# Luca96/carla-driving-rl-agent

Measured on AMD Instinct MI355X. Metric: PPO update-steps/sec (batch=256, 4x90x120x3 obs), higher is better.
Workload: dtype f32; 1 GPU; configs[1]: synthetic rollout buffer 256x4-frame 90x120x3 obs per GPU, full CARLANetwork fwd/bwd + PPO (re-sampled Beta, pathwise) / value loss + clip + Adam, fp32; per_gpu_batch=256, global_batch=256, parallelism=dp1, policy_loss=resampled (reference-faithful)

## Files before the change

carla-driving-rl-agent_amd/csrc/gemm_pw_bwd.hip:

```cpp
#include <stdlib.h>

#include "colreduce.h"

namespace cdrl {

typedef float f32x16 __attribute__((ext_vector_type(16)));
typedef __bf16 bf16x8 __attribute__((ext_vector_type(8)));
typedef __bf16 bf16x4 __attribute__((ext_vector_type(4)));
typedef uint32_t u32x2 __attribute__((ext_vector_type(2)));
typedef float f32x2 __attribute__((ext_vector_type(2)));

struct PwbArgs {
    View dz;
    int dz_shuffle;
    int act;
    const float* y;
    const float* stats;
    const float* coef;
    View a;
    const float* a_stats;
    const __bf16* Wp;
    int wp_ks;
    View da;
    float* qpart;
// ... 471 lines not shown
                int dc = shuffle_dst(a.dz.coff + c0 + h, a.dz_shuffle);
                if (dc + 1 >= a.dz.ld) {
                    dc -= 1;
                    hi_half[h] = true;
                }
                vo[h] = cok[h] ? (uint32_t)((4 * rg) * a.dz.ld + dc) * 2u : OOR;
            }
        } else {
            vo[0] = cok[0] ? (uint32_t)((4 * rg) * a.dz.ld + a.dz.coff + c0) * 2u : OOR;
            vo[1] = cok[2] ? (uint32_t)((4 * rg) * a.dz.ld + a.dz.coff + c0 + 2) * 2u : OOR;
        }
        voy[0] = cok[0] ? (uint32_t)((4 * rg) * N + c0) * 2u : OOR;
        voy[1] = cok[2] ? (uint32_t)((4 * rg) * N + c0 + 2) * 2u : OOR;
        const __amdgpu_buffer_rsrc_t rsD = __builtin_amdgcn_make_buffer_rsrc(a.dz.p, 0, (int)(Mtot * a.dz.ld * 2), 0x00020000);
        const __amdgpu_buffer_rsrc_t rsY = __builtin_amdgcn_make_buffer_rsrc(const_cast<float*>(a.y), 0, (int)(Mtot * N * 2), 0x00020000);
        const uint32_t rowD = (uint32_t)a.dz.ld * 2u, rowY = (uint32_t)N * 2u;
        const bool relu6 = a.act == ACT_RELU6;
        uint32_t rz[4][2], ry[4][2];
        auto load_row = [&](int t, int j) {
            const int64_t m0 = mbeg + (int64_t)t * BM;
            const uint32_t mu = (uint32_t)m0;
            const int left = (int)(mend - (m0 + 4 * rg));
            const uint32_t msk = j < left ? 0u : OOR;
#pragma unroll
            for (int h = 0; h < 2; ++h) {
                rz[j][h] = __builtin_amdgcn_raw_buffer_load_b32(rsD, (vo[h] + (uint32_t)j * rowD) | msk, mu * rowD, 0);
                ry[j][h] = __builtin_amdgcn_raw_buffer_load_b32(rsY, (voy[h] + (uint32_t)j * rowY) | msk, mu * rowY, 0);
            }
        };
        double cs[4] = {0.0, 0.0, 0.0, 0.0};
        auto store_tile = [&](int t) {
            const bool more = t + 1 < t1;
            const int left = (int)(mend - (mbeg + (int64_t)t * BM + 4 * rg));
            f32x2 cmean[2], cinv[2], csc[2], csh[2], ck1[2], ck2[2], ck3[2];
            {
                const float4 q0 = *reinterpret_cast<const float4*>(&cf[0 * NP + c0]), q1 = *reinterpret_cast<const float4*>(&cf[1 * NP + c0]);
                const float4 q2 = *reinterpret_cast<const float4*>(&cf[2 * NP + c0]), q3 = *reinterpret_cast<const float4*>(&cf[3 * NP + c0]);
                const float4 q4 = *reinterpret_cast<const float4*>(&cf[4 * NP + c0]), q5 = *reinterpret_cast<const float4*>(&cf[5 * NP + c0]);
                const float4 q6 = *reinterpret_cast<const float4*>(&cf[6 * NP + c0]);
                cmean[0] = f32x2{q0.x, q0.y}; cmean[1] = f32x2{q0.z, q0.w};
                cinv[0] = f32x2{q1.x, q1.y}; cinv[1] = f32x2{q1.z, q1.w};
                csc[0] = f32x2{q2.x, q2.y}; csc[1] = f32x2{q2.z, q2.w};
                csh[0] = f32x2{q3.x, q3.y}; csh[1] = f32x2{q3.z, q3.w};
                ck1[0] = f32x2{q4.x, q4.y}; ck1[1] = f32x2{q4.z, q4.w};
                ck2[0] = f32x2{q5.x, q5.y}; ck2[1] = f32x2{q5.z, q5.w};
                ck3[0] = f32x2{q6.x, q6.y}; ck3[1] = f32x2{q6.z, q6.w};
            }
            uint32_t hw[4][2];
            f32x2 ts[2] = {f32x2{0.0f, 0.0f}, f32x2{0.0f, 0.0f}};
#pragma unroll
            for (int j = 0; j < 4; ++j) {
                const bool rok = j < left;
                f32x2 dz2[2];
                if (SHUF) {
                    const f32x2 pa = widen(hi_half[0] ? rz[j][0] >> 16 : rz[j][0]), pb = widen(hi_half[1] ? rz[j][1] >> 16 : rz[j][1]);
                    dz2[0] = f32x2{pa[0], pb[0]};
                    dz2[1] = f32x2{pa[1], pb[1]};
                    if (!cok[2]) dz2[1][0] = 0.0f;
                    if (!cok[3]) dz2[1][1] = 0.0f;
                } else {
                    dz2[0] = widen(rz[j][0]);
                    dz2[1] = widen(rz[j][1]);
                }
                f32x2 vrow[2];
#pragma unroll
                for (int h = 0; h < 2; ++h) {
                    f32x2 d = dz2[h];
                    const f32x2 yv = widen(ry[j][h]);
                    if (relu6) {
                        const f32x2 z = __builtin_elementwise_fma(csc[h], yv, csh[h]);
                        if (!relu6_open(z[0])) d[0] = 0.0f;
                        if (!relu6_open(z[1])) d[1] = 0.0f;
                    }
                    const f32x2 xh = (yv - cmean[h]) * cinv[h];
                    f32x2 v = ck1[h] * (d - ck2[h] - xh * ck3[h]);
                    if (!rok) v = f32x2{0.0f, 0.0f};
                    vrow[h] = v;
                }
                if (more) load_row(t + 1, j);
#pragma unroll
                for (int h = 0; h < 2; ++h) {
                    ts[h] += vrow[h];
                    hw[j][h] = pack(vrow[h]);
                }
                *reinterpret_cast<u32x2*>(&Rm[(4 * rg + j) * LDR + c0]) = u32x2{hw[j][0], hw[j][1]};
            }
            cs[0] += (double)ts[0][0];
            cs[1] += (double)ts[0][1];
            cs[2] += (double)ts[1][0];
            cs[3] += (double)ts[1][1];
#pragma unroll
            for (int h = 0; h < 2; ++h) {
                *reinterpret_cast<u32x2*>(&Dt[(c0 + 2 * h) * LDT + 4 * rg]) = u32x2{pwb_lolo(hw[0][h], hw[1][h]), pwb_lolo(hw[2][h], hw[3][h])};
                *reinterpret_cast<u32x2*>(&Dt[(c0 + 2 * h + 1) * LDT + 4 * rg]) = u32x2{pwb_hihi(hw[0][h], hw[1][h]), pwb_hihi(hw[2][h], hw[3][h])};
            }
        };
        const __amdgpu_buffer_rsrc_t rsC = __builtin_amdgcn_make_buffer_rsrc(a.da.p, 0, (int)(Mtot * a.da.ld * 2), 0x00020000);
        const uint32_t rowC = (uint32_t)a.da.ld * 2u;
        const int ncol = dwc * 32 + lrow;
        const bool odd = (lane & 1) != 0;
        const uint32_t voC = (ncol & ~1) < K ? (uint32_t)((4 * lk + (odd ? 1 : 0)) * a.da.ld + a.da.coff + (ncol & ~1)) * 2u : OOR;
        auto swap1 = [](float x) -> float { return __int_as_float(__builtin_amdgcn_mov_dpp(__float_as_int(x), 0xB1, 0xF, 0xF, true)); };
        double sda = 0.0, sdx = 0.0;
        auto compute_tile = [&](int t) {
            f32x16 acc;
#pragma unroll
            for (int r = 0; r < 16; ++r) acc[r] = 0.0f;
            const int64_t m0 = mbeg + (int64_t)t * BM + dwr * 32;
            const uint32_t mu = (uint32_t)m0;
            const int left = (int)(mend - m0) - 4 * lk - (odd ? 1 : 0);
            uint32_t cold[ACC ? 8 : 1];
            if (ACC) {
#pragma unroll
                for (int q = 0; q < 8; ++q) {
                    const int rr = ((2 * q) & 3) + 8 * ((2 * q) >> 2);
                    cold[ACC ? q : 0] = __builtin_amdgcn_raw_buffer_load_b32(rsC, voC | (rr < left ? 0u : OOR), (mu + (uint32_t)rr) * rowC, 0);
                }
            }
            const int ao = (dwr * 32 + lrow) * LDR + 8 * lk;
#pragma unroll
            for (int s = 0; s < KS_DA; ++s) {
                const bf16x8 a1 = *reinterpret_cast<const bf16x8*>(&Rm[ao + 16 * s]);
                const bf16x8 b1 = *reinterpret_cast<const bf16x8*>(&Wl[((s * 2 + lk) * 128 + ncol) * 8]);
                acc = __builtin_amdgcn_mfma_f32_32x32x16_bf16(a1, b1, acc, 0, 0, 0);
            }
            if (ANORM) {
                const int xo = ncol * LDT + dwr * 32 + 4 * lk;
#pragma unroll
                for (int i = 0; i < 4; ++i) {
                    const u32x2 xw = *reinterpret_cast<const u32x2*>(&At[xo + 8 * i]);
                    const f32x2 x01 = widen(xw[0]), x23 = widen(xw[1]);
                    sda += ((double)acc[4 * i] + (double)acc[4 * i + 1]) + ((double)acc[4 * i + 2] + (double)acc[4 * i + 3]);
                    sdx += ((double)acc[4 * i] * (double)x01[0] + (double)acc[4 * i + 1] * (double)x01[1]) +
                           ((double)acc[4 * i + 2] * (double)x23[0] + (double)acc[4 * i + 3] * (double)x23[1]);
                }
            }
#pragma unroll
            for (int q = 0; q < 8; ++q) {
                const float recv = swap1(odd ? acc[2 * q] : acc[2 * q + 1]);
                float lo = odd ? recv : acc[2 * q], hi = odd ? acc[2 * q + 1] : recv;
                if (ACC) {
                    lo += bf_lo(cold[ACC ? q : 0]);
                    hi += bf_hi(cold[ACC ? q : 0]);
                }
                const int rr = ((2 * q) & 3) + 8 * ((2 * q) >> 2);
                __builtin_amdgcn_raw_buffer_store_b32(bf_pack(lo, hi), rsC, voC | (rr < left ? 0u : OOR), (mu + (uint32_t)rr) * rowC, 0);
            }
        };
        if (t0 < t1) {
#pragma unroll
            for (int j = 0; j < 4; ++j) load_row(t0, j);
        }
        __syncthreads();
        for (int t = t0; t < t1; ++t) {
            store_tile(t);
            __syncthreads();
            compute_tile(t);
            __syncthreads();
        }
        double* red = reinterpret_cast<double*>(smem_raw);
#pragma unroll
        for (int e = 0; e < 4; ++e) red[rg * NP + c0 + e] = cs[e];
        __syncthreads();
        for (int c = tid; c < NP; c += 256) {
            double s = 0.0;
#pragma unroll
            for (int r = 0; r < NRG; ++r) s += red[r * NP + c];
            a.dbpart[((int64_t)g * a.nbpg + b) * NP + c] = s;
        }
        if (ANORM && a.spart) {
            __syncthreads();
            double* r2 = reinterpret_cast<double*>(smem_raw);
            r2[((dwr * 2 + lk) * 2 + 0) * KP + ncol] = sda;
            r2[((dwr * 2 + lk) * 2 + 1) * KP + ncol] = sdx;
            __syncthreads();
            for (int i = tid; i < 2 * KP; i += 256) {
                const int q = i / KP, c = i % KP;
                double s = 0.0;
#pragma unroll
                for (int w = 0; w < DA_WR * 2; ++w) s += r2[(w * 2 + q) * KP + c];
                a.spart[(((int64_t)g * a.nbpg + b) * 2 + q) * KP + c] = s;
            }
        }
    } else {
        const int qw = wave & 3;
        const int qkt = qw % Q_KT, qnt0 = (qw / Q_KT) * NTW;
        f32x2 cmean[2] = {f32x2{0.0f, 0.0f}, f32x2{0.0f, 0.0f}}, cinv[2] = {f32x2{0.0f, 0.0f}, f32x2{0.0f, 0.0f}};
        if (ANORM) {
            const int GK = a.G * K;
#pragma unroll
            for (int e = 0; e < 4; ++e) {
                const int c = c0 + e;
                const bool on = c < K;
                cmean[e >> 1][e & 1] = on ? a.a_stats[0 * GK + g * K + (on ? c : 0)] : 0.0f;
                cinv[e >> 1][e & 1] = on ? a.a_stats[1 * GK + g * K + (on ? c : 0)] : 0.0f;
            }
        }
        uint32_t vo[2];
        vo[0] = c0 < K ? (uint32_t)((4 * rg) * a.a.ld + a.a.coff + c0) * 2u : OOR;
        vo[1] = c0 + 2 < K ? (uint32_t)((4 * rg) * a.a.ld + a.a.coff + c0 + 2) * 2u : OOR;
        const __amdgpu_buffer_rsrc_t rsA = __builtin_amdgcn_make_buffer_rsrc(a.a.p, 0, (int)(Mtot * a.a.ld * 2), 0x00020000);
        const uint32_t rowA = (uint32_t)a.a.ld * 2u;
        uint32_t rz[4][2];
        auto load_row = [&](int t, int j) {
            const int64_t m0 = mbeg + (int64_t)t * BM;
            const uint32_t mu = (uint32_t)m0;
            const int left = (int)(mend - (m0 + 4 * rg));
            const uint32_t msk = j < left ? 0u : OOR;
#pragma unroll
            for (int h = 0; h < 2; ++h) rz[j][h] = __builtin_amdgcn_raw_buffer_load_b32(rsA, (vo[h] + (uint32_t)j * rowA) | msk, mu * rowA, 0);
        };
        auto store_tile = [&](int t) {
            const bool more = t + 1 < t1;
            const int left = (int)(mend - (mbeg + (int64_t)t * BM + 4 * rg));
            uint32_t hw[4][2];
#pragma unroll
            for (int j = 0; j < 4; ++j) {
                const bool rok = j < left;
                if (ANORM) {
#pragma unroll
                    for (int h = 0; h < 2; ++h) {
                        f32x2 v = (widen(rz[j][h]) - cmean[h]) * cinv[h];
                        if (!rok) v = f32x2{0.0f, 0.0f};
                        hw[j][h] = pack(v);
                    }
                } else {
                    hw[j][0] = rz[j][0];
                    hw[j][1] = rz[j][1];
                }
                if (more) load_row(t + 1, j);
            }
#pragma unroll
            for (int h = 0; h < 2; ++h) {
                *reinterpret_cast<u32x2*>(&At[(c0 + 2 * h) * LDT + 4 * rg]) = u32x2{pwb_lolo(hw[0][h], hw[1][h]), pwb_lolo(hw[2][h], hw[3][h])};
                *reinterpret_cast<u32x2*>(&At[(c0 + 2 * h + 1) * LDT + 4 * rg]) = u32x2{pwb_hihi(hw[0][h], hw[1][h]), pwb_hihi(hw[2][h], hw[3][h])};
            }
        };
        f32x16 qacc[NTW];
#pragma unroll
        for (int j = 0; j < NTW; ++j)
#pragma unroll
            for (int r = 0; r < 16; ++r) qacc[j][r] = 0.0f;
        auto compute_tile = [&]() {
            const int ao = (qkt * 32 + lrow) * LDT + 8 * lk;
#pragma unroll
            for (int s = 0; s < KS_Q; ++s) {
                const bf16x8 a1 = *reinterpret_cast<const bf16x8*>(&At[ao + 16 * s]);
#pragma unroll
                for (int j = 0; j < NTW; ++j) {
                    const bf16x8 d1 = *reinterpret_cast<const bf16x8*>(&Dt[((qnt0 + j) * 32 + lrow) * LDT + 8 * lk + 16 * s]);
                    qacc[j] = __builtin_amdgcn_mfma_f32_32x32x16_bf16(a1, d1, qacc[j], 0, 0, 0);
                }
            }
        };
        if (t0 < t1) {
#pragma unroll
            for (int j = 0; j < 4; ++j) load_row(t0, j);
        }
        __syncthreads();
        for (int t = t0; t < t1; ++t) {
            store_tile(t);
            __syncthreads();
            compute_tile();
            __syncthreads();
        }
        float* qp = a.qpart + ((int64_t)g * a.nbpg + b) * KP * NP;
#pragma unroll
        for (int j = 0; j < NTW; ++j) {
            const int n = (qnt0 + j) * 32 + lrow;
#pragma unroll
            for (int r = 0; r < 16; ++r) {
                const int k = qkt * 32 + (r & 3) + 8 * (r >> 2) + 4 * lk;
                qp[k * NP + n] = qacc[j][r];
            }
        }
        __syncthreads();
        if (ANORM && a.spart) {
            __syncthreads();
            __syncthreads();
        }
    }
}

struct PwbReduceArgs {
    const float* qpart;
    const double* dbpart;
    const double* spart;
    const float* W;
    const float* a_stats;
    const float* a_gamma;
    const float* a_beta;
    float* dW;
    float* db;
    float* a_dgamma;
    float* a_dbeta;
    float* a_coef;
    const double* fin_tot;
    float* o_dgamma;
    float* o_dbeta;
    int N, K, KP, NP, G, Mg, nbpg;
    int wbf;
};

constexpr int PWB_RS = 8;
__global__ void __launch_bounds__(128 * PWB_RS) pwb_reduce_kernel(PwbReduceArgs a) {
    __shared__ double sq[PWB_RS][128];
    __shared__ double sd[PWB_RS][128];
    __shared__ double red[2][8][2];
    const int k = blockIdx.x, n = threadIdx.x & 127, sl = threadIdx.x >> 7;
    const int N = a.N, K = a.K, G = a.G;
    const bool on = n < N;
    const int nsl = PWB_RS / G > 0 ? PWB_RS / G : 1;
    const int per = (a.nbpg + nsl - 1) / nsl;
    for (int pair = sl; pair < G * nsl; pair += PWB_RS) {
        const int g = pair % G, s = pair / G;
        const int b0 = s * per, b1 = min(a.nbpg, b0 + per);
        double q = 0.0, d = 0.0;
        if (on) {
            const float* pq = a.qpart + ((int64_t)g * a.nbpg * a.KP + k) * a.NP + n;
            const double* pd = a.dbpart + (int64_t)g * a.nbpg * a.NP + n;
            int b = b0;
            const bool need_d = a.a_stats != nullptr || k == 0;
            for (; b + 32 <= b1; b += 32) {
                float v[32];
                double u[32];
#pragma unroll
                for (int i = 0; i < 32; ++i) {
                    v[i] = pq[(int64_t)(b + i) * a.KP * a.NP];
                    u[i] = need_d ? pd[(int64_t)(b + i) * a.NP] : 0.0;
                }
#pragma unroll
                for (int i = 0; i < 32; ++i) {
                    q += (double)v[i];
                    d += u[i];
                }
            }
            for (; b + 16 <= b1; b += 16) {
                float v[16];
                double u[16];
#pragma unroll
                for (int i = 0; i < 16; ++i) {
                    v[i] = pq[(int64_t)(b + i) * a.KP * a.NP];
                    u[i] = pd[(int64_t)(b + i) * a.NP];
                }
#pragma unroll
                for (int i = 0; i < 16; ++i) {
                    q += (double)v[i];
                    d += u[i];
                }
            }
            for (; b + 8 <= b1; b += 8) {
                float v[8];
                double u[8];
#pragma unroll
                for (int i = 0; i < 8; ++i) {
                    v[i] = pq[(int64_t)(b + i) * a.KP * a.NP];
                    u[i] = pd[(int64_t)(b + i) * a.NP];
                }
#pragma unroll
                for (int i = 0; i < 8; ++i) {
                    q += (double)v[i];
                    d += u[i];
                }
            }
            for (; b < b1; ++b) {
                q += (double)pq[(int64_t)b * a.KP * a.NP];
                d += pd[(int64_t)b * a.NP];
            }
        }
        sq[pair][n] = q;
        sd[pair][n] = d;
    }
    __syncthreads();
    const bool lead = sl == 0;
    float w = (on && lead) ? a.W[(int64_t)k * N + n] : 0.0f;
    if (a.wbf) w = (float)(__bf16)w;
    double qtot = 0.0, dbtot = 0.0;
    double s1[8], s2[8];
#pragma unroll
    for (int g = 0; g < 8; ++g) {
        s1[g] = s2[g] = 0.0;
        if (g < G && lead) {
            double q = sq[g][n], d = sd[g][n];
            for (int s = 1; s < nsl; ++s) {
                q += sq[s * G + g][n];
                d += sd[s * G + g][n];
            }
            qtot += q;
            dbtot += d;
            s1[g] = (double)w * d;
            s2[g] = (double)w * q;
        }
    }
    if (on && lead) {
        if (a.a_stats) a.dW[(int64_t)k * N + n] = (float)((double)a.a_gamma[k] * qtot + (double)a.a_beta[k] * dbtot);
        else a.dW[(int64_t)k * N + n] = (float)qtot;
        if (k == 0) a.db[n] = (float)dbtot;
        if (k == 0 && a.fin_tot) {
            double dg = 0.0, dbt = 0.0;
            for (int g = 0; g < G; ++g) {
                dbt += a.fin_tot[((int64_t)g * 2 + 0) * N + n];
                dg += a.fin_tot[((int64_t)g * 2 + 1) * N + n];
            }
            a.o_dgamma[n] = (float)dg;
            a.o_dbeta[n] = (float)dbt;
        }
    }
    if (!a.a_stats) return;
    const int lane = n & 63, wave = n >> 6;
#pragma unroll
    for (int g = 0; g < 8; ++g) {
        if (g >= G) break;
        double u1 = s1[g], u2 = s2[g];
#pragma unroll
        for (int o = 32; o > 0; o >>= 1) {
            u1 += __shfl_down(u1, o);
            u2 += __shfl_down(u2, o);
        }
        if (lane == 0 && lead) {
            red[0][g][wave] = u1;
            red[1][g][wave] = u2;
        }
    }
    __syncthreads();
    if (a.spart && (int)(threadIdx.x >> 6) < 2 * G) {
        const int pr = threadIdx.x >> 6, g = pr >> 1, q = pr & 1, l = threadIdx.x & 63;
        double u = 0.0;
        for (int b = l; b < a.nbpg; b += 64) u += a.spart[(((int64_t)g * a.nbpg + b) * 2 + q) * a.KP + k];
#pragma unroll
        for (int o = 32; o > 0; o >>= 1) u += __shfl_down(u, o);
        if (l == 0) {
            red[q][g][0] = u;
            red[q][g][1] = 0.0;
        }
    }
    __syncthreads();
    if (threadIdx.x == 0) {
        const int GK = G * K;
        const double cnt = (double)a.Mg;
        double dg = 0.0, dbt = 0.0;
        for (int g = 0; g < G; ++g) {
            const double u1 = red[0][g][0] + red[0][g][1], u2 = red[1][g][0] + red[1][g][1];
            dbt += u1;
            dg += u2;
            a.a_coef[0 * GK + g * K + k] = a.a_stats[2 * GK + g * K + k];
            a.a_coef[1 * GK + g * K + k] = (float)(u1 / cnt);
            a.a_coef[2 * GK + g * K + k] = (float)(u2 / cnt);
        }
        a.a_dgamma[k] = (float)dg;
        a.a_dbeta[k] = (float)dbt;
    }
}

static inline int pwb_pad(int c) { return c <= 64 ? 64 : 128; }

bool pw_bwd_fused_supported(View dz, View a, View da, int N, int K, int at) {
    if (N > 128 || K > 128 || N < 8 || K < 8 || (N & 1) || (K & 1)) return false;
    if (at && pwb_pad(N) != pwb_pad(K)) return false;
    if (pwb_pad(N) != pwb_pad(K) && !(pwb_pad(K) == 64 && pwb_pad(N) == 128)) return false;
    auto ok = [](View v) { return (v.ld % 2 == 0) && (v.coff % 2 == 0) && ((reinterpret_cast<uintptr_t>(v.p) & 7) == 0); };
    return ok(a) && ok(da) && (dz.ld % 2 == 0) && ((reinterpret_cast<uintptr_t>(dz.p) & 7) == 0);
}

int pw_bwd_fused_nbpg(int G, int Mg, int N, int K, int at) {
    const int bm = (pwb_pad(K) == 128 || pwb_pad(N) == 128) ? 32 : 64;
    const int tiles = cdiv(Mg, bm);
    int nb = 256 / G;
    if (at && tiles >= 6 * (512 / G)) nb = 512 / G;
    if (nb < 1) nb = 1;
    return nb > tiles ? tiles : nb;
}

int64_t pw_bwd_fused_qpart_elems(int G, int Mg, int N, int K, int at) {
    return (int64_t)G * pw_bwd_fused_nbpg(G, Mg, N, K, at) * pwb_pad(K) * pwb_pad(N);
}

int64_t pw_bwd_fused_dbpart_elems(int G, int Mg, int N, int K, int at) {
    return (int64_t)G * pw_bwd_fused_nbpg(G, Mg, N, K, at) * pwb_pad(N) * (at ? 3 : 1);
}

template <int KP, int NP, bool SHUF, bool ANORM, bool ACC>
static int pwb_launch(const PwbArgs& a, hipStream_t st) {
    constexpr int BM = (KP == 128 || NP == 128) ? 32 : 64;
    constexpr size_t lds = (size_t)(3 * BM * (NP + 8) + 3 * (NP + KP) * (BM + 8)) * 2 + (size_t)7 * NP * sizeof(float);
    auto kern = pwb_kernel<KP, NP, SHUF, ANORM, ACC>;
    static LdsAttrOnce attr;
    if (attr.need()) {
        CDRL_HIP(hipFuncSetAttribute(reinterpret_cast<const void*>(kern), hipFuncAttributeMaxDynamicSharedMemorySize, (int)lds));
        attr.mark();
    }
    hipLaunchKernelGGL(kern, dim3(a.G * a.nbpg), dim3(512), lds, st, a);
    CDRL_LAUNCH_CHECK();
    return 0;
}

template <int P, bool SHUF, bool ANORM, bool ACC>
static int pwb16_launch(const PwbArgs& a, hipStream_t st) {
    constexpr int BM = P == 128 ? 32 : 64;
    constexpr size_t lds = (size_t)(BM * (P + 8) + 2 * P * (BM + 8)) * 2 + (size_t)7 * P * sizeof(float) + (size_t)(P / 16) * 2 * 128 * 8 * 2;
    auto kern = pwb16_kernel<P, P, SHUF, ANORM, ACC>;
    static LdsAttrOnce attr;
    if (attr.need() && lds >= 64 * 1024) {
        CDRL_HIP(hipFuncSetAttribute(reinterpret_cast<const void*>(kern), hipFuncAttributeMaxDynamicSharedMemorySize, (int)lds));
        attr.mark();
    }
    hipLaunchKernelGGL(kern, dim3(a.G * a.nbpg), dim3(512), lds, st, a);
    CDRL_LAUNCH_CHECK();
    return 0;
}

template <int P, bool SHUF>
static int pwb16_launch2(const PwbArgs& a, bool anorm, bool acc, hipStream_t st) {
    if (anorm) return acc ? pwb16_launch<P, SHUF, true, true>(a, st) : pwb16_launch<P, SHUF, true, false>(a, st);
    return acc ? pwb16_launch<P, SHUF, false, true>(a, st) : pwb16_launch<P, SHUF, false, false>(a, st);
}

template <int KP, int NP, bool SHUF>
static int pwb_launch2(const PwbArgs& a, bool anorm, bool acc, hipStream_t st) {
    if (anorm) return acc ? pwb_launch<KP, NP, SHUF, true, true>(a, st) : pwb_launch<KP, NP, SHUF, true, false>(a, st);
    return acc ? pwb_launch<KP, NP, SHUF, false, true>(a, st) : pwb_launch<KP, NP, SHUF, false, false>(a, st);
}

int pw_bwd_fused(const PwBwdFused& f, hipStream_t st) {
    if (!pw_bwd_fused_supported(f.dz, f.a, f.da, f.N, f.K, f.at) || !f.Wp) {
        set_error("pw_bwd_fused: unsupported shape / alignment N=%d K=%d", f.N, f.K);
        return -1;
    }
    const int64_t Mtot = (int64_t)f.G * f.Mg;
    if (f.at && ((f.dz.coff | f.dz.ld | f.a.coff | f.a.ld | f.da.coff | f.da.ld) & 1)) {
        set_error("pw_bwd_fused: bf16 storage needs even leading dimensions / channel offsets");
        return -1;
    }
    if (Mtot * f.dz.ld * 4 >= ((int64_t)1 << 31) || Mtot * f.a.ld * 4 >= ((int64_t)1 << 31) || Mtot * f.N * 4 >= ((int64_t)1 << 31) ||
        Mtot * f.da.ld * 4 >= ((int64_t)1 << 31)) {
        set_error("pw_bwd_fused: operand of 2 GB or more");
        return -1;
    }
    if (f.G > 8) {
        set_error("pw_bwd_fused: more than 8 groups");
        return -1;
    }
    PwbArgs a;
    a.dz = f.dz;
    a.dz_shuffle = f.dz_shuffle;
    a.act = f.act;
    a.y = f.y;
    a.stats = f.stats;
    a.coef = f.coef;
    a.a = f.a;
    a.a_stats = f.a_stats;
    a.Wp = reinterpret_cast<const __bf16*>(f.Wp);
    a.wp_ks = pw_x3_ksteps(f.N);
    a.da = f.da;
    a.qpart = f.qpart;
    a.dbpart = f.dbpart;
    a.N = f.N;
    a.K = f.K;
    a.G = f.G;
    a.Mg = f.Mg;
    a.nbpg = pw_bwd_fused_nbpg(f.G, f.Mg, f.N, f.K, f.at);
    a.at = f.at;
    a.fin_part = f.at ? nullptr : f.fin_part;
    a.fin_tot = f.fin_tot;
    a.fin_nb = f.fin_nb;
    if (f.fin_part && (f.at || !f.fin_tot || f.fin_nb <= 0)) {
        set_error("pw_bwd_fused: finalize-on-load needs the float32 form, fin_tot and fin_nb");
        return -1;
    }
    a.spart = (f.at && f.a_stats) ? f.dbpart + (int64_t)f.G * a.nbpg * pwb_pad(f.N) : nullptr;
    static const int dbg = cdrl_getenv("CDRL_DIAG_PWB") ? atoi(cdrl_getenv("CDRL_DIAG_PWB")) : 0;
    a.dbg = dbg;
    const bool anorm = f.a_stats != nullptr, acc = f.accumulate != 0, shuf = f.dz_shuffle != 0;
    if (f.at && pwb_pad(f.K) != pwb_pad(f.N)) {
        set_error("pw_bwd_fused: the bf16-storage form is instantiated for equal paddings only (N=%d K=%d)", f.N, f.K);
        return -1;
    }
    if (f.at) {
        if (pwb_pad(f.K) == 128) return shuf ? pwb16_launch2<128, true>(a, anorm, acc, st) : pwb16_launch2<128, false>(a, anorm, acc, st);
        return shuf ? pwb16_launch2<64, true>(a, anorm, acc, st) : pwb16_launch2<64, false>(a, anorm, acc, st);
    }
    if (pwb_pad(f.K) == 128) return shuf ? pwb_launch2<128, 128, true>(a, anorm, acc, st) : pwb_launch2<128, 128, false>(a, anorm, acc, st);
    if (pwb_pad(f.N) == 128) return shuf ? pwb_launch2<64, 128, true>(a, anorm, acc, st) : pwb_launch2<64, 128, false>(a, anorm, acc, st);
    return shuf ? pwb_launch2<64, 64, true>(a, anorm, acc, st) : pwb_launch2<64, 64, false>(a, anorm, acc, st);
}

int pw_bwd_fused_reduce(const PwBwdFused& f, hipStream_t st) {
    PwbReduceArgs r;
    r.qpart = f.qpart;
    r.dbpart = f.dbpart;
    r.W = f.W;
    r.a_stats = f.a_stats;
    r.a_gamma = f.a_gamma;
    r.a_beta = f.a_beta;
    r.dW = f.dW;
    r.db = f.db;
    r.a_dgamma = f.a_dgamma;
    r.a_dbeta = f.a_dbeta;
    r.a_coef = f.a_coef;
    r.N = f.N;
    r.K = f.K;
    r.KP = pwb_pad(f.K);
    r.NP = pwb_pad(f.N);
    r.G = f.G;
    r.Mg = f.Mg;
    r.nbpg = pw_bwd_fused_nbpg(f.G, f.Mg, f.N, f.K, f.at);
    r.wbf = f.at;
    r.fin_tot = (f.fin_part && !f.at) ? f.fin_tot : nullptr;
    r.o_dgamma = f.o_dgamma;
    r.o_dbeta = f.o_dbeta;
    if (r.fin_tot && (!f.o_dgamma || !f.o_dbeta)) {
        set_error("pw_bwd_fused_reduce: finalize-on-load needs the dgamma / dbeta outputs of the BatchNorm behind the conv");
        return -1;
    }
    r.spart = (f.at && f.a_stats) ? f.dbpart + (int64_t)f.G * r.nbpg * pwb_pad(f.N) : nullptr;
    if (f.a_stats && (!f.a_gamma || !f.a_beta || !f.a_dgamma || !f.a_dbeta || !f.a_coef)) {
        set_error("pw_bwd_fused_reduce: normalised input needs gamma / beta and the dgamma / dbeta / coef outputs");
        return -1;
    }
    hipLaunchKernelGGL(pwb_reduce_kernel, dim3(f.K), dim3(128 * PWB_RS), 0, st, r);
    CDRL_LAUNCH_CHECK();
    return 0;
}

}
```

Before: 79.60 update-steps/s.

## Split pointwise-backward reduce into plain and normalised-input kernels

Measured after the change: 79.55 update-steps/s, median of 2. No clear change (-0.1%).

```diff
diff --git a/carla-driving-rl-agent_amd/csrc/gemm_pw_bwd.hip b/carla-driving-rl-agent_amd/csrc/gemm_pw_bwd.hip
--- a/carla-driving-rl-agent_amd/csrc/gemm_pw_bwd.hip
+++ b/carla-driving-rl-agent_amd/csrc/gemm_pw_bwd.hip
@@ -797,85 +797,130 @@
     int wbf;
 };
 
+template <int U, bool D>
+__device__ __forceinline__ void pwb_slot_round(const float* pq, int64_t sq, const double* pd, int64_t sd, uint32_t n, int& b, int b1, double& q, double& d) {
+    for (; b + U <= b1; b += U) {
+        float v[U];
+        double u[U];
+#pragma unroll
+        for (int i = 0; i < U; ++i) {
+            v[i] = (pq + (int64_t)(b + i) * sq)[n];
+            if (D) u[i] = (pd + (int64_t)(b + i) * sd)[n];
+        }
+#pragma unroll
+        for (int i = 0; i < U; ++i) {
+            q += (double)v[i];
+            if (D) d += u[i];
+        }
+    }
+}
+
+template <bool D>
+__device__ __forceinline__ void pwb_slot_sum(const float* pq, int64_t sq, const double* pd, int64_t sd, uint32_t n, int b0, int b1, double& q, double& d) {
+    int b = b0;
+    pwb_slot_round<32, D>(pq, sq, pd, sd, n, b, b1, q, d);
+    pwb_slot_round<16, D>(pq, sq, pd, sd, n, b, b1, q, d);
+    pwb_slot_round<8, D>(pq, sq, pd, sd, n, b, b1, q, d);
+    pwb_slot_round<1, D>(pq, sq, pd, sd, n, b, b1, q, d);
+}
+
 constexpr int PWB_RS = 8;
+
+constexpr int PWB_NC = 32;
+__global__ void __launch_bounds__(PWB_NC * PWB_RS) pwb_reduce_plain_kernel(PwbReduceArgs a) {
+    __shared__ double sq[PWB_RS][PWB_NC];
+    __shared__ double sd[PWB_RS][PWB_NC];
+    const int k = blockIdx.x, nl = threadIdx.x % PWB_NC, n = blockIdx.y * PWB_NC + nl, pair = threadIdx.x / PWB_NC;
+    const int N = a.N, G = a.G;
+    const bool on = n < N;
+    const int nsl = PWB_RS / G > 0 ? PWB_RS / G : 1;
+    const int per = (a.nbpg + nsl - 1) / nsl;
+    const bool need_d = k == 0;
+    if (pair < G * nsl) {
+        const int g = pair % G, s = pair / G;
+        const int b0 = s * per, b1 = min(a.nbpg, b0 + per);
+        double q = 0.0, d = 0.0;
+        if (on) {
+            const float* pq = a.qpart + ((int64_t)g * a.nbpg * a.KP + k) * a.NP;
+            const double* pd = a.dbpart + (int64_t)g * a.nbpg * a.NP;
+            if (need_d) pwb_slot_sum<true>(pq, (int64_t)a.KP * a.NP, pd, a.NP, n, b0, b1, q, d);
+            else pwb_slot_sum<false>(pq, (int64_t)a.KP * a.NP, pd, a.NP, n, b0, b1, q, d);
+        }
+        sq[pair][nl] = q;
+        sd[pair][nl] = d;
+    }
+    __syncthreads();
+    if (pair != 0 || !on) return;
+    double qtot = 0.0, dbtot = 0.0;
+    for (int g = 0; g < G; ++g) {
+        double q = sq[g][nl], d = sd[g][nl];
+        for (int s = 1; s < nsl; ++s) {
+            q += sq[s * G + g][nl];
+            d += sd[s * G + g][nl];
+        }
+        qtot += q;
+        dbtot += d;
+    }
+    a.dW[(int64_t)k * N + n] = (float)qtot;
+    if (!need_d) return;
+    a.db[n] = (float)dbtot;
+    if (a.fin_tot) {
+        double dg = 0.0, dbt = 0.0;
+        for (int g = 0; g < G; ++g) {
+            dbt += a.fin_tot[((int64_t)g * 2 + 0) * N + n];
+            dg += a.fin_tot[((int64_t)g * 2 + 1) * N + n];
+        }
+        a.o_dgamma[n] = (float)dg;
+        a.o_dbeta[n] = (float)dbt;
+    }
+}
+
 __global__ void __launch_bounds__(128 * PWB_RS) pwb_reduce_kernel(PwbReduceArgs a) {
     __shared__ double sq[PWB_RS][128];
     __shared__ double sd[PWB_RS][128];
     __shared__ double red[2][8][2];
-    const int k = blockIdx.x, n = threadIdx.x & 127, sl = threadIdx.x >> 7;
-    const int N = a.N, K = a.K, G = a.G;
+    const int k = blockIdx.x, n = threadIdx.x & 127;
+    const int pair = threadIdx.x >> 7;
+    const int N = a.N, K = a.K, G = a.G, GK = G * K;
     const bool on = n < N;
     const int nsl = PWB_RS / G > 0 ? PWB_RS / G : 1;
     const int per = (a.nbpg + nsl - 1) / nsl;
-    for (int pair = sl; pair < G * nsl; pair += PWB_RS) {
+    float w = (on && pair < G) ? a.W[(int64_t)k * N + n] : 0.0f;
+    const float gam = a.a_gamma[k], bet = a.a_beta[k];
+    if (pair < G * nsl) {
         const int g = pair % G, s = pair / G;
         const int b0 = s * per, b1 = min(a.nbpg, b0 + per);
         double q = 0.0, d = 0.0;
-        if (on) {
-            const float* pq = a.qpart + ((int64_t)g * a.nbpg * a.KP + k) * a.NP + n;
-            const double* pd = a.dbpart + (int64_t)g * a.nbpg * a.NP + n;
-            int b = b0;
-            const bool need_d = a.a_stats != nullptr || k == 0;
-            for (; b + 32 <= b1; b += 32) {
-                float v[32];
-                double u[32];
-#pragma unroll
-                for (int i = 0; i < 32; ++i) {
-                    v[i] = pq[(int64_t)(b + i) * a.KP * a.NP];
-                    u[i] = need_d ? pd[(int64_t)(b + i) * a.NP] : 0.0;
-                }
-#pragma unroll
-                for (int i = 0; i < 32; ++i) {
-                    q += (double)v[i];
-                    d += u[i];
-                }
-            }
-            for (; b + 16 <= b1; b += 16) {
-                float v[16];
-                double u[16];
-#pragma unroll
-                for (int i = 0; i < 16; ++i) {
-                    v[i] = pq[(int64_t)(b + i) * a.KP * a.NP];
-                    u[i] = pd[(int64_t)(b + i) * a.NP];
-                }
-#pragma unroll
-                for (int i = 0; i < 16; ++i) {
-                    q += (double)v[i];
-                    d += u[i];
-                }
-            }
-            for (; b + 8 <= b1; b += 8) {
-                float v[8];
-                double u[8];
-#pragma unroll
-                for (int i = 0; i < 8; ++i) {
-                    v[i] = pq[(int64_t)(b + i) * a.KP * a.NP];
-                    u[i] = pd[(int64_t)(b + i) * a.NP];
-                }
-#pragma unroll
-                for (int i = 0; i < 8; ++i) {
-                    q += (double)v[i];
-                    d += u[i];
-                }
-            }
-            for (; b < b1; ++b) {
-                q += (double)pq[(int64_t)b * a.KP * a.NP];
-                d += pd[(int64_t)b * a.NP];
-            }
-        }
+        if (on)
+            pwb_slot_sum<true>(a.qpart + ((int64_t)__builtin_amdgcn_readfirstlane(g) * a.nbpg * a.KP + k) * a.NP, (int64_t)a.KP * a.NP,
+                               a.dbpart + (int64_t)g * a.nbpg * a.NP, a.NP, n, b0, b1, q, d);
         sq[pair][n] = q;
         sd[pair][n] = d;
     }
     __syncthreads();
-    const bool lead = sl == 0;
-    float w = (on && lead) ? a.W[(int64_t)k * N + n] : 0.0f;
-    if (a.wbf) w = (float)(__bf16)w;
-    double qtot = 0.0, dbtot = 0.0;
-    double s1[8], s2[8];
-#pragma unroll
-    for (int g = 0; g < 8; ++g) {
-        s1[g] = s2[g] = 0.0;
-        if (g < G && lead) {
+    const float k1 = (int)threadIdx.x < G ? a.a_stats[2 * GK + threadIdx.x * K + k] : 0.0f;
+    if (pair < G) {
+        const int g = pair;
+        if (a.wbf) w = (float)(__bf16)w;
+        double q = sq[g][n], d = sd[g][n];
+        for (int s = 1; s < nsl; ++s) {
+            q += sq[s * G + g][n];
+            d += sd[s * G + g][n];
+        }
+        double u1 = (double)w * d, u2 = (double)w * q;
+#pragma unroll
+        for (int o = 32; o > 0; o >>= 1) {
+            u1 += __shfl_down(u1, o);
+            u2 += __shfl_down(u2, o);
+        }
+        if ((n & 63) == 0) {
+            red[0][g][n >> 6] = u1;
+            red[1][g][n >> 6] = u2;
+        }
+    }
+    if (pair == PWB_RS - 1 && on) {
+        double qtot = 0.0, dbtot = 0.0;
+        for (int g = 0; g < G; ++g) {
             double q = sq[g][n], d = sd[g][n];
             for (int s = 1; s < nsl; ++s) {
                 q += sq[s * G + g][n];
@@ -883,13 +928,8 @@
             }
             qtot += q;
             dbtot += d;
-            s1[g] = (double)w * d;
-            s2[g] = (double)w * q;
-        }
-    }
-    if (on && lead) {
-        if (a.a_stats) a.dW[(int64_t)k * N + n] = (float)((double)a.a_gamma[k] * qtot + (double)a.a_beta[k] * dbtot);
-        else a.dW[(int64_t)k * N + n] = (float)qtot;
+        }
+        a.dW[(int64_t)k * N + n] = (float)((double)gam * qtot + (double)bet * dbtot);
         if (k == 0) a.db[n] = (float)dbtot;
         if (k == 0 && a.fin_tot) {
             double dg = 0.0, dbt = 0.0;
@@ -901,46 +941,34 @@
             a.o_dbeta[n] = (float)dbt;
         }
     }
-    if (!a.a_stats) return;
-    const int lane = n & 63, wave = n >> 6;
-#pragma unroll
-    for (int g = 0; g < 8; ++g) {
-        if (g >= G) break;
-        double u1 = s1[g], u2 = s2[g];
-#pragma unroll
-        for (int o = 32; o > 0; o >>= 1) {
-            u1 += __shfl_down(u1, o);
-            u2 += __shfl_down(u2, o);
-        }
-        if (lane == 0 && lead) {
-            red[0][g][wave] = u1;
-            red[1][g][wave] = u2;
-        }
-    }
     __syncthreads();
-    if (a.spart && (int)(threadIdx.x >> 6) < 2 * G) {
-        const int pr = threadIdx.x >> 6, g = pr >> 1, q = pr & 1, l = threadIdx.x & 63;
-        double u = 0.0;
-        for (int b = l; b < a.nbpg; b += 64) u += a.spart[(((int64_t)g * a.nbpg + b) * 2 + q) * a.KP + k];
-#pragma unroll
-        for (int o = 32; o > 0; o >>= 1) u += __shfl_down(u, o);
-        if (l == 0) {
-            red[q][g][0] = u;
-            red[q][g][1] = 0.0;
-        }
-    }
-    __syncthreads();
+    if (a.spart) {
+        if ((int)(threadIdx.x >> 6) < 2 * G) {
+            const int pr = threadIdx.x >> 6, g = pr >> 1, q = pr & 1, l = threadIdx.x & 63;
+            double u = 0.0;
+            for (int b = l; b < a.nbpg; b += 64) u += a.spart[(((int64_t)g * a.nbpg + b) * 2 + q) * a.KP + k];
+#pragma unroll
+            for (int o = 32; o > 0; o >>= 1) u += __shfl_down(u, o);
+            if (l == 0) {
+                red[q][g][0] = u;
+                red[q][g][1] = 0.0;
+            }
+        }
+        __syncthreads();
+    }
+    const double cnt = (double)a.Mg;
+    if ((int)threadIdx.x < G) {
+        const int g = threadIdx.x;
+        const double u1 = red[0][g][0] + red[0][g][1], u2 = red[1][g][0] + red[1][g][1];
+        a.a_coef[0 * GK + g * K + k] = k1;
+        a.a_coef[1 * GK + g * K + k] = (float)(u1 / cnt);
+        a.a_coef[2 * GK + g * K + k] = (float)(u2 / cnt);
+    }
     if (threadIdx.x == 0) {
-        const int GK = G * K;
-        const double cnt = (double)a.Mg;
         double dg = 0.0, dbt = 0.0;
         for (int g = 0; g < G; ++g) {
-            const double u1 = red[0][g][0] + red[0][g][1], u2 = red[1][g][0] + red[1][g][1];
-            dbt += u1;
-            dg += u2;
-            a.a_coef[0 * GK + g * K + k] = a.a_stats[2 * GK + g * K + k];
-            a.a_coef[1 * GK + g * K + k] = (float)(u1 / cnt);
-            a.a_coef[2 * GK + g * K + k] = (float)(u2 / cnt);
+            dbt += red[0][g][0] + red[0][g][1];
+            dg += red[1][g][0] + red[1][g][1];
         }
         a.a_dgamma[k] = (float)dg;
         a.a_dbeta[k] = (float)dbt;
@@ -1112,7 +1140,8 @@
         set_error("pw_bwd_fused_reduce: normalised input needs gamma / beta and the dgamma / dbeta / coef outputs");
         return -1;
     }
-    hipLaunchKernelGGL(pwb_reduce_kernel, dim3(f.K), dim3(128 * PWB_RS), 0, st, r);
+    if (f.a_stats) hipLaunchKernelGGL(pwb_reduce_kernel, dim3(f.K), dim3(128 * PWB_RS), 0, st, r);
+    else hipLaunchKernelGGL(pwb_reduce_plain_kernel, dim3(f.K, cdiv(f.N, PWB_NC)), dim3(PWB_NC * PWB_RS), 0, st, r);
     CDRL_LAUNCH_CHECK();
     return 0;
 }
```
